# mourisl/T1K

Hardware: AMD Instinct MI355X
Metric: genotyped reads/sec (end-to-end genotyper stage, 2x150 bp HLA) (higher is better)
Workload: dtype u64

## Files before the change

### t1k_amd/csrc/t1k_assign.hip

```cpp
#include "t1k_dev.h"
#include "t1k_launch.h"
#include "t1k_memo.h"

#define WG 256
#define GA_BIG_MAX 2048
#define GA_SCRATCH_INTS (6 * (GA_BIG_MAX + 4))

enum { ERR_HITCAP = 1, ERR_STAGECAP = 2, ERR_CANDCAP = 4, ERR_BIGGROUP = 8, ERR_OVLCAP = 16, ERR_SORTCAP = 32, ERR_SLOWCAP = 64, ERR_ROWCAP = 128, ERR_GROUPCAP = 256 };

__global__ void k_pack_reads(const char *ascii, const uint64_t *offs, uint32_t n, int S, uint64_t *bases, uint64_t *nmask, uint16_t *lens, int nCode) {
  uint64_t gid = (uint64_t)blockIdx.x * blockDim.x + threadIdx.x;
  uint64_t total = (uint64_t)n * S;
  if (gid >= total) return;
  uint32_t re = (uint32_t)(gid / S);
  int w = (int)(gid % S);
  uint64_t o = offs[re];
  int len = (int)(offs[re + 1] - o);
  if (w == 0) lens[re] = (uint16_t)len;
  uint64_t fb = 0, fn = 0, rb = 0, rn = 0;
  for (int q = 0; q < 32; ++q) {
    int i = w * 32 + q;
    if (i >= len) break;
    char c = ascii[o + i];
    int code = c == 'A' ? 0 : c == 'C' ? 1 : c == 'G' ? 2 : c == 'T' ? 3 : 4;
// ... 338 lines not shown
#define SEL_F_EXTOK 2u
#define SEL_F_KEEPCLIP 4u
__device__ __forceinline__ bool packSelectKey(const KeyW &W, int m, int d, int rspan, uint32_t allele, uint32_t index, uint32_t flags, int aBits, int iBits, uint64_t *out) {
  const int MMAX = (1 << W.MB) - 1, DMAX = (1 << W.DB) - 1, RMAX = (1 << W.RB) - 1;
  if (m < 0 || m > MMAX || d < 0 || d > DMAX || rspan < 0 || rspan > RMAX || 1 + W.MB + W.DB + W.RB + 3 + aBits + iBits > 64) return false;
  *out = ((((((uint64_t)(MMAX - m) << W.DB | (uint64_t)d) << W.RB | (uint64_t)(RMAX - rspan)) << aBits | (uint64_t)allele) << iBits) | (uint64_t)index) << 3 | flags;
  return true;
}

__device__ inline bool candBeforeFull(const T1kCand &a, const T1kCand &b) {
  int ars = a.readSE & 0xFFFF, are = a.readSE >> 16, brs = b.readSE & 0xFFFF, bre = b.readSE >> 16;
  if (ars != brs) return ars < brs;
  if (are != bre) return are < bre;
  if (a.seqStart != b.seqStart) return a.seqStart < b.seqStart;
  return a.seqEnd < b.seqEnd;
}

#define SELECT_SMALL 2048
#define SELECT_LARGE 8192

#ifndef T1K_SELECT_SMALL_WAVES
#define T1K_SELECT_SMALL_WAVES 7
#endif
template <int SELECT_LDS_CAP, int NT, bool XL>
__global__ __launch_bounds__(NT) __attribute__((amdgpu_waves_per_eu(SELECT_LDS_CAP == SELECT_SMALL ? T1K_SELECT_SMALL_WAVES : 8))) void k_select(SelectArgs P) {
  extern __shared__ uint64_t dynLds[];
  uint64_t *sKey = dynLds;
  __shared__ uint32_t warpSums[NT / 64];
  __shared__ int sLatch, sGood, sBest, sTie;
  __shared__ uint32_t sBase;
  __shared__ CsTables sCs;
  __shared__ uint16_t sCnt[256 * (NT / 64)];
  const int tid = threadIdx.x;
  unsigned int nbTotal = 0;
  __shared__ uint32_t sNextRe;
  uint32_t hoNext = 0, hoLeft = 0;
  for (;;) {
    __syncthreads();
    if (tid == 0) {
      constexpr uint32_t HO = SELECT_LDS_CAP == SELECT_SMALL ? T1K_SELECT_SMALL_HANDOUT : T1K_SELECT_LARGE_HANDOUT;
      if (hoLeft == 0) { hoNext = (uint32_t)atomicAdd(&P.counters[SELECT_LDS_CAP == SELECT_SMALL ? 28 : 29], (unsigned long long)HO); hoLeft = HO; }
      sNextRe = hoNext++; --hoLeft;
    }
    __syncthreads();
    const uint32_t re = sNextRe;
    if (re >= P.reads.nReadEnds) break;
    const uint32_t n = P.candCount[re], c0 = P.candStart[re];
    if (n == 0) {
      if (tid == 0 && SELECT_LDS_CAP == SELECT_SMALL) { P.ovlStart[re] = 0; P.ovlCount[re] = 0; }
      continue;
    }
    if ((n > SELECT_SMALL) != (SELECT_LDS_CAP == SELECT_LARGE)) continue;
    const uint32_t live = n;
    if (live == 0) {
      if (tid == 0) { P.ovlStart[re] = 0; P.ovlCount[re] = 0; }
      continue;
    }
    uint32_t np2 = 8;
    while (np2 < live) np2 <<= 1;
    uint64_t *key;
    if (np2 <= SELECT_LDS_CAP) key = sKey;
    else if (np2 <= P.sortCap) key = P.sortScratch + (uint64_t)blockIdx.x * P.sortCap * 6;
    else {
      if (tid == 0) { atomicOr(&P.counters[2], (unsigned long long)ERR_SORTCAP); P.ovlStart[re] = 0; P.ovlCount[re] = 0; }
      continue;
    }
    int iBits = 1;
    while ((1u << iBits) < n) ++iBits;
    const uint64_t iMask = (1ull << iBits) - 1;
    const KeyW W = selectWidths<XL>((int)P.reads.len[re]);
    const int mShift = W.DB + W.RB + P.alleleBits + iBits + 3;
    const int mMax = (1 << W.MB) - 1;
    auto idxOf = [&](uint64_t kk) { return (uint32_t)((kk >> 3) & iMask); };
    auto seedOf = [&](uint64_t kk) { return mMax - (int)((kk >> mShift) & (uint64_t)mMax); };
    for (uint32_t i = live + tid; i < np2; i += NT) key[i] = ~0ull;
    for (uint32_t i = tid; i < n; i += NT) {
      const uint16_t fl = P.ext[c0 + i].flags;
      const T1kCand c = P.cand[c0 + i];
      int rs = c.readSE & 0xFFFF, rend = c.readSE >> 16;
      int m = (int)(c.match >> 16);
      int rspan = rend - rs, d = rspan + 1 + c.seqEnd - c.seqStart + 1;
      const double sim = (double)m / (double)(c.seqEnd - c.seqStart + 1 + rend - rs + 1);
      const uint32_t kf = ((fl & T1K_F_SEPSEED) ? SEL_F_SEPSEED : 0u) | ((fl & T1K_F_EXTOK) ? SEL_F_EXTOK : 0u) |
                          (((fl & T1K_F_NEEDCLIP) && !(sim < 0.95)) ? SEL_F_KEEPCLIP : 0u);
      const uint32_t slot = i;
      uint64_t kk;
      if (!packSelectKey(W, m, d, rspan, c.allele & 0x7FFFFFFFu, i, kf, P.alleleBits, iBits, &kk)) { atomicOr(&P.counters[2], (unsigned long long)ERR_SORTCAP); kk = (uint64_t)i << 3; }
// ... 42 lines not shown
    __syncthreads();
    if (tid == 0) sGood = sFirst == 0x7FFFFFFF ? -1 : seedOf(key[sFirst]);
    __syncthreads();
    const int good = sGood;
    uint32_t written = 0;
    unsigned int nbLocal = 0;
    int myBest = -1;
    uint32_t mine = 0;
    for (uint32_t i = tid; i < live; i += NT) {
      const uint64_t kk = key[i];
      const uint32_t fl = (uint32_t)kk & 7u;
      bool emit = false;
      if (!(fl & SEL_F_SEPSEED)) {
        bool tried = true;
        if ((int)i > latch && seedOf(kk) < good && !(fl & SEL_F_KEEPCLIP)) tried = false;
        emit = tried && (fl & SEL_F_EXTOK);
        if (emit) { const int xm = (int)P.ext[c0 + idxOf(kk)].matchCnt; if (xm > myBest) myBest = xm; }
      }
      if (emit) { ++mine; key[i] = kk | (1ull << 63); }
    }
    atomicMax(&sBest, myBest);
    uint32_t tot;
    t1k_block_scan_exclusive_n<NT / 64>(mine, warpSums, &tot);
    if (tid == 0) {
      unsigned long long b = atomicAdd(&P.counters[1], (unsigned long long)tot);
      if (b + tot > P.ovlCap) { atomicOr(&P.counters[2], (unsigned long long)ERR_OVLCAP); sBase = 0xFFFFFFFFu; P.ovlStart[re] = 0; P.ovlCount[re] = 0; }
      else { sBase = (uint32_t)b; P.ovlStart[re] = (uint32_t)b; P.ovlCount[re] = tot; }
    }
    __syncthreads();
    const int bestMatch = sBest;
    if (sBase != 0xFFFFFFFFu) {
      for (uint32_t i0 = 0; i0 < live; i0 += NT) {
        uint32_t i = i0 + tid;
        uint32_t flag = (i < live && (key[i] >> 63)) ? 1u : 0u;
        uint32_t t2;
        uint32_t off = t1k_block_scan_exclusive_n<NT / 64>(flag, warpSums, &t2);
        if (flag) {
          uint32_t ci = c0 + idxOf(key[i]);
          const T1kCand c = P.cand[ci];
          const T1kExt x = P.ext[ci];
          T1kOvl o;
          o.allele = c.allele & 0x7FFFFFFFu;
          o.seqStart = x.seqStart; o.seqEnd = x.seqEnd; o.readStart = x.readStart; o.readEnd = x.readEnd;
          o.matchCnt = x.matchCnt; o.leftClip = x.leftClip; o.rightClip = x.rightClip; o.re = re;
          o.flags = ((int)x.matchCnt >= bestMatch - 10 ? 1u : 0u) | ((c.allele >> 31) ? 0u : 2u);
          o.relaxed = (!P.relax && (o.flags & 1)) ? x.matchCnt : (uint16_t)0;
          if (o.flags & 1) ++nbLocal;
          P.ovl[(uint64_t)sBase + written + off] = o;
        }
        written += t2;
      }
    }
    nbTotal += nbLocal;
    __syncthreads();
  }
  t1k_stat_add(P.counters, T1K_STAT_NEARBEST, nbTotal);
}


__global__ __launch_bounds__(WG) void k_fullalign(FullArgs P) {
  uint64_t gid = (uint64_t)blockIdx.x * blockDim.x + threadIdx.x;
  if (gid >= P.nOvl) return;
  T1kOvl o = P.ovl[gid];
  if (!(o.flags & 1)) { P.ovl[gid].relaxed = 0; return; }
  const int pass = (o.flags & 2) ? 1 : 0;
  const int S = P.reads.S;
  const uint64_t *rb = P.reads.bases + ((uint64_t)o.re * 2 + pass) * S;
  const uint64_t *rn = P.reads.nmask + ((uint64_t)o.re * 2 + pass) * S;
  const int64_t goff = (int64_t)P.ref.alleleOff[o.allele];
  const int L = o.readEnd - o.readStart + 1, Ls = o.seqEnd - o.seqStart + 1;
  const int w = P.noCov ? 0 : (P.undo ? -(int)P.reads.weight[o.re] : (int)P.reads.weight[o.re]);
  bool slow = (L != Ls) || L > T1K_MAX_READ_LEN;
  int x = 0, exonMis = 0;
  uint64_t covw[10];
  if (!slow && L <= 160) {
    typedef uint64_t u64x2 __attribute__((ext_vector_type(2), aligned(8)));
    uint64_t gB[6], gN[6], rB[6], rN[6], gE[6];
    const int64_t gpos = goff + o.seqStart;
// ... 447 lines not shown
    __syncthreads();
    if (threadIdx.x == 0) sCarry += (int32_t)tot;
    __syncthreads();
  }
}

int t1k_launch_pack(t1k_ctx *ctx, const char *dAscii, const uint64_t *dOffs, uint32_t n, int S, uint64_t *bases, uint64_t *nmask, uint16_t *lens, int nCode) {
  uint64_t total = (uint64_t)n * S;
  if (!total) return 0;
  hipLaunchKernelGGL(k_pack_reads, dim3((unsigned)((total + 255) / 256)), dim3(256), 0, ctx->stream, dAscii, dOffs, n, S, bases, nmask, lens, nCode);
  return 0;
}

size_t t1k_slow_per_thread(int maxCells) { return (size_t)GA_SCRATCH_INTS * 4 + 4224 + (size_t)maxCells + 64; }

void t1k_launch_extend(t1k_ctx *ctx, const ExtendArgs &a) {
  if (!a.nCand) return;
  hipLaunchKernelGGL(k_extend, dim3((unsigned)((a.nCand + WG - 1) / WG)), dim3(WG), 0, ctx->stream, a);
}
void t1k_launch_extend_retry_dev(t1k_ctx *ctx, const ExtendArgs &a, const uint32_t *list, int arena, uint64_t est) {
  const unsigned long long *nDev = (const unsigned long long *)ctx->bCounters.p + T1K_TOTAL_BASE + arena;
  hipLaunchKernelGGL(k_extend_retry, dim3((unsigned)std::max<uint64_t>(1, (est + WG - 1) / WG)), dim3(WG), 0, ctx->stream, a, list, 0u, nDev);
}
void t1k_launch_select(t1k_ctx *ctx, const SelectArgs &a, int nWg) {
  if (a.xl) {
    hipFuncSetAttribute((const void *)k_select<SELECT_LARGE, 1024, true>, hipFuncAttributeMaxDynamicSharedMemorySize, SELECT_LARGE * 8);
    hipLaunchKernelGGL((k_select<SELECT_SMALL, 256, true>), dim3(nWg), dim3(256), SELECT_SMALL * 8, ctx->stream, a);
    hipLaunchKernelGGL((k_select<SELECT_LARGE, 1024, true>), dim3(std::min(nWg, 512)), dim3(1024), SELECT_LARGE * 8, ctx->stream, a);
    return;
  }
  hipFuncSetAttribute((const void *)k_select<SELECT_LARGE, 1024, false>, hipFuncAttributeMaxDynamicSharedMemorySize, SELECT_LARGE * 8);
  hipLaunchKernelGGL((k_select<SELECT_SMALL, 256, false>), dim3(nWg), dim3(256), SELECT_SMALL * 8, ctx->stream, a);
  hipLaunchKernelGGL((k_select<SELECT_LARGE, 1024, false>), dim3(std::min(nWg, 512)), dim3(1024), SELECT_LARGE * 8, ctx->stream, a);
}
void t1k_launch_fullalign(t1k_ctx *ctx, const FullArgs &a) {
  if (!a.nOvl) return;
  hipLaunchKernelGGL(k_fullalign, dim3((unsigned)((a.nOvl + WG - 1) / WG)), dim3(WG), 0, ctx->stream, a);
}
void t1k_launch_fullalign_slow(t1k_ctx *ctx, const SlowArgs &a, int nBlocks) { hipLaunchKernelGGL(k_fullalign_slow, dim3(nBlocks * 64), dim3(64), 0, ctx->stream, a); }
void t1k_launch_align_flags(t1k_ctx *ctx, const SlowArgs &a, uint32_t *flags) {
  hipLaunchKernelGGL(k_align_flags, dim3((a.nSlow + WG - 1) / WG), dim3(WG), 0, ctx->stream, a, flags);
}
void t1k_launch_align_reps(t1k_ctx *ctx, const uint32_t *flags, const uint32_t *runOf, uint32_t *rep, uint32_t n) {
  hipLaunchKernelGGL(k_align_reps, dim3((n + WG - 1) / WG), dim3(WG), 0, ctx->stream, flags, runOf, rep, n);
}
void t1k_launch_align_fill_apply(t1k_ctx *ctx, const SlowArgs &a, bool eq) {
  if (eq) {
    hipLaunchKernelGGL(k_align_fill<true>, dim3((a.nRuns + WG - 1) / WG), dim3(WG), 0, ctx->stream, a);
    hipLaunchKernelGGL(k_align_apply_eq, dim3((a.nSlow + WG - 1) / WG), dim3(WG), 0, ctx->stream, a);
  } else {
    hipLaunchKernelGGL(k_align_fill<false>, dim3((a.nRuns + WG - 1) / WG), dim3(WG), 0, ctx->stream, a);
    hipLaunchKernelGGL(k_align_apply_band, dim3((a.nSlow + WG - 1) / WG), dim3(WG), 0, ctx->stream, a);
  }
}
void t1k_launch_truncate(t1k_ctx *ctx, const TruncArgs &a, int nWg) {
  if (a.xl) {
// ... 96 lines not shown
```

### t1k_amd/csrc/t1k_capi.hip

```cpp
#include <sys/mman.h>
#include <map>
#include <mutex>
#include <unordered_map>
#include <algorithm>
#include <memory>
#include <thread>
#include <chrono>
#include <cstring>
#include <cstdio>
#include <cstdlib>
#include "t1k_dev.h"
#include "t1k_launch.h"

namespace {
struct DevPool {
  std::mutex m;
  std::map<int, std::multimap<size_t, void *>> freeBlocks;
  std::unordered_map<void *, std::pair<size_t, int>> live;
  size_t pooled = 0;
};
DevPool &devPool() { static DevPool *p = new DevPool(); return *p; }
}

hipError_t t1k_dev_malloc(void **out, size_t bytes) {
// ... 754 lines not shown
      const uint64_t before = ctx->wGroup;
      grow(ctx->wGroup, ctx->needGroup, ctx->prm.group_cap);
      if (ctx->wGroup > before && !ctx->scaledOnce) {
        const double f = std::min(4.0, (double)ctx->wGroup / (double)before);
        ctx->wList = std::min<uint64_t>((uint64_t)ctx->prm.group_cap, (uint64_t)(ctx->wList * f));
        ctx->wCand = std::min<uint64_t>((uint64_t)ctx->prm.cand_cap, (uint64_t)(ctx->wCand * f));
        ctx->wOvl = std::min<uint64_t>((uint64_t)ctx->prm.ovl_cap, (uint64_t)(ctx->wOvl * f));
        ctx->scaledOnce = true;
      }
      grow(ctx->wList, ctx->needList, ctx->prm.group_cap);
      grow(ctx->wRare, ctx->needRare, ctx->prm.group_cap);
      grow(ctx->wJob, ctx->needJob, jobLimit * 2);
      grow(ctx->wGenJob, ctx->needGenJob, jobLimit * 2);
    }
    if (ctx->lastCapFlags & 2) grow(ctx->wGenHit, ctx->needGenHit, genHitLimit);
    if (ctx->lastCapFlags & 4) grow(ctx->wCand, ctx->needCand, ctx->prm.cand_cap);
    if (ctx->lastCapFlags & 16) grow(ctx->wOvl, ctx->needOvl, ctx->prm.ovl_cap);
    if (ctx->lastCapFlags & 64) grew = true;
    if (!grew || (ctx->lastCapFlags & ~(256ull | 4ull | 16ull | 64ull | 2ull))) return rc;
    if (getenv("T1K_DEBUG_PHASES")) fprintf(stderr, "[t1k] range of %u read-ends again with capacities: groups %llu lists %llu / %llu jobs %llu / %llu candidates %llu overlaps %llu\n", count,
                                            (unsigned long long)ctx->wGroup, (unsigned long long)ctx->wList, (unsigned long long)ctx->wRare, (unsigned long long)ctx->wJob, (unsigned long long)ctx->wGenJob,
                                            (unsigned long long)ctx->wCand, (unsigned long long)ctx->wOvl);
  }
}

static int assignOnce(t1k_ctx *ctx, uint64_t first, uint32_t count) {
  const uint32_t n = count;
  ctx->covCommitted = false;
  T1kReadsDev rd = ctx->reads;
  rd.nReadEnds = count;
  rd.bases += first * 2 * rd.S; rd.nmask += first * 2 * rd.S; rd.len += first; rd.weight += first;
  if (rd.skip) rd.skip += first;
  ctx->rangeCount = count;
  int rc;
  const int nWg = (int)std::min<uint32_t>((uint32_t)ctx->prm.workgroups, std::max<uint32_t>(n, 1));
  const uint32_t sortCap = 1u << 15;
  const int maxChunks = t1k_chain_max_chunks(ctx->ref.nAlleles), memoN = t1k_chain_memo_entries();
  const bool longReads = ctx->batchFastMaxLen > 160;
  const int recStride = t1k_chain_rec_stride(ctx->batchFastMaxLen);
  const uint64_t groupCap = ctx->wGroup;
  const uint32_t jobCap = (uint32_t)ctx->wJob, genCandCap = 16u << 20, genHitCap = (uint32_t)std::min<uint64_t>(ctx->wGenHit ? ctx->wGenHit : (64u << 20), 1024u << 20), genJobCap = (uint32_t)ctx->wGenJob;
  const int bigBlocks = 32;
  if ((rc = t1k_ensure(ctx, ctx->bCounters, (size_t)T1K_COUNTER_WORDS * 8))) return rc;
  if ((rc = t1k_ensure(ctx, ctx->bWgGroups, groupCap * recStride * 4))) return rc;
  if ((rc = t1k_ensure(ctx, ctx->bWgStage, (size_t)n * maxChunks * 8 + 64))) return rc;
  const int maxK = t1k_chain_max_kmers(ctx->batchMaxLen, ctx->prm.kmer_length);
// ... 5 lines not shown
  const uint32_t jobSegCap = jobCap / T1K_NSTRIPE, genCandSegCap = genCandCap / T1K_NSTRIPE;
  const size_t listWords = (size_t)listSegCap * T1K_NSTRIPE, rareWords = (size_t)rareSegCap * T1K_NSTRIPE;
  if ((rc = t1k_ensure(ctx, ctx->bLists, ((size_t)jobCap * 2 + listWords * 5 + rareWords * 6 + (size_t)genCandCap * 6 + genHitCap + (size_t)genJobCap * 2) * 4 + 64))) return rc;
  if ((rc = t1k_ensure(ctx, ctx->bCand, (size_t)ctx->wCand * sizeof(T1kCand)))) return rc;
  if ((rc = t1k_ensure(ctx, ctx->bExt, (size_t)ctx->wCand * sizeof(T1kExt)))) return rc;
  const uint64_t chunkEntries = std::max<uint64_t>(ctx->wOvl, (uint64_t)std::max(1, ctx->prm.store_chunk_mb) * ((1ull << 20) / sizeof(T1kOvlP)));
  {
    const int sl = ctx->storeSlot;
    std::vector<T1kDevBuf> &chunks = ctx->storeChunks[sl];
    for (;;) {
      if (ctx->storeChunk[sl] >= chunks.size()) chunks.resize(ctx->storeChunk[sl] + 1);
      T1kDevBuf &ch = chunks[ctx->storeChunk[sl]];
      if (ch.p && ctx->storeUsed[sl] + ctx->wOvl <= ch.bytes / sizeof(T1kOvlP)) break;
      if (ch.p && ctx->storeUsed[sl] > 0) { ++ctx->storeChunk[sl]; ctx->storeUsed[sl] = 0; continue; }
      if (ch.p) { (void)t1k_dev_free(ch.p); ch.p = nullptr; ch.bytes = 0; }
      const auto t0 = std::chrono::steady_clock::now();
      hipError_t e = t1k_dev_malloc(&ch.p, chunkEntries * sizeof(T1kOvlP));
      ctx->msAlloc += std::chrono::duration<double, std::milli>(std::chrono::steady_clock::now() - t0).count(); ctx->bytesAlloc += chunkEntries * sizeof(T1kOvlP);
      if (e != hipSuccess) { ch.p = nullptr; return t1k_fail(ctx, T1K_ERR_DEVICE, std::string("overlap store: hipMalloc of another ") + std::to_string(chunkEntries * sizeof(T1kOvlP) >> 20) + " MB chunk failed (" + hipGetErrorString(e) + "); fewer fragments per window (T1K_WINDOW) need less"); }
      ch.bytes = chunkEntries * sizeof(T1kOvlP);
    }
    ctx->storeBase = (T1kOvlP *)chunks[ctx->storeChunk[sl]].p + ctx->storeUsed[sl];
  }
  if ((rc = t1k_ensure(ctx, ctx->bOvlWork, (size_t)ctx->wOvl * sizeof(T1kOvl)))) return rc;
  ctx->ovlBase = (T1kOvl *)ctx->bOvlWork.p;
  if ((rc = t1k_ensure(ctx, ctx->bCandStart, (size_t)(n + 1) * 4))) return rc;
  if ((rc = t1k_ensure(ctx, ctx->bCandCount, (size_t)(n + 1) * 4))) return rc;
  if ((rc = t1k_ensure(ctx, ctx->bOvlStart, (size_t)(n + 1) * 4))) return rc;
  if ((rc = t1k_ensure(ctx, ctx->bOvlCount, (size_t)(n + 1) * 4))) return rc;
  if ((rc = t1k_ensure(ctx, ctx->bSortScratch, (size_t)std::min(nWg, 512) * sortCap * 48))) return rc;
  T1K_HIP(ctx, hipMemsetAsync(ctx->bCounters.p, 0, (size_t)T1K_COUNTER_WORDS * 8, ctx->stream));
  T1K_HIP(ctx, hipMemsetAsync(ctx->bOvlCount.p, 0, (size_t)n * 4 + 4, ctx->stream));
  T1K_HIP(ctx, hipMemsetAsync(ctx->bCandCount.p, 0, (size_t)n * 4 + 4, ctx->stream));
  T1K_HIP(ctx, hipMemsetAsync(ctx->bWgCache.p, 0, (size_t)n * memoN * 8, ctx->stream));
  ctx->nCand = ctx->nOvl = 0;
  ctx->traceFetch = 0;
  if (getenv("T1K_DEBUG_TRACE")) fprintf(stderr, "[t1k trace] assign_range first %llu count %u\n", (unsigned long long)first, n);
  memset(&ctx->stats, 0, sizeof(ctx->stats));
  if (n == 0) return T1K_OK;
  unsigned long long hc[64];
  double t0 = nowMs();
  ChainArgs a{};
  a.ref = ctx->ref; a.reads = rd;
  a.k = ctx->prm.kmer_length; a.radius = ctx->prm.radius; a.hitLenRequired = ctx->prm.hit_len_required;
  a.sim = ctx->prm.ref_seq_similarity;
  const int relaxFlag = ctx->prm.relax_intron_align;
  a.recs = (uint32_t *)ctx->bWgGroups.p; a.recStride = (uint32_t)recStride; a.groupCap = groupCap;
  a.chunkStart = (uint32_t *)ctx->bWgStage.p; a.chunkCount = a.chunkStart + (size_t)n * maxChunks; a.maxChunks = maxChunks;
// ... 22 lines not shown
  ctx->nCand = hc[0];
  ExtendArgs e{};
  e.ref = ctx->ref; e.reads = rd; e.k = a.k; e.sim = a.sim;
  e.cand = a.cand; e.ext = (T1kExt *)ctx->bExt.p; e.nCand = ctx->nCand; e.counters = a.counters;
  e.memo = a.memo; e.jobStr = a.jobStr; e.jobSegCap = a.jobSegCap; e.retryStr = a.retryStr; e.retrySegCap = a.listSegCap;
  t1k_launch_extend(ctx, e);
  if (ctx->nCand) {
    const uint64_t jobCapAll = (uint64_t)e.jobSegCap * T1K_NSTRIPE, retryCapAll = (uint64_t)e.retrySegCap * T1K_NSTRIPE;
    const uint64_t eJ = t1k_arena_estimate(ctx, T1K_AR_EXTJOBS, jobCapAll, n), eR = t1k_arena_estimate(ctx, T1K_AR_EXTRETRY, retryCapAll, n);
    t1k_arena_compact_dev(ctx, T1K_AR_EXTJOBS, e.jobStr, e.jobSegCap, a.jobList, eJ);
    t1k_arena_compact_dev(ctx, T1K_AR_EXTRETRY, e.retryStr, e.retrySegCap, a.retryList, eR);
    t1k_launch_dp_dense_dev(ctx, a, a.jobList, T1K_AR_EXTJOBS, (uint32_t)jobCapAll, eJ);
    t1k_launch_extend_retry_dev(ctx, e, a.retryList, T1K_AR_EXTRETRY, eR);
  }
  T1K_HIP(ctx, hipEventRecord(ctx->ev[2], ctx->stream));
  double t2 = nowMs();
  SelectArgs s{};
  s.reads = rd; s.cand = a.cand; s.ext = e.ext; s.candStart = a.candStart; s.candCount = a.candCount;
  s.ovl = ctx->ovlBase; s.ovlCap = ctx->wOvl;
  s.ovlStart = (uint32_t *)ctx->bOvlStart.p; s.ovlCount = (uint32_t *)ctx->bOvlCount.p;
  s.sortScratch = (uint64_t *)ctx->bSortScratch.p; s.sortCap = sortCap; s.counters = a.counters;
  s.alleleBits = 1; s.relax = relaxFlag; s.xl = ctx->batchMaxLen > T1K_MAX_READ_LEN ? 1 : 0;
  while ((1u << s.alleleBits) < ctx->ref.nAlleles) ++s.alleleBits;
  t1k_launch_select(ctx, s, nWg);
  T1K_HIP(ctx, hipEventRecord(ctx->ev[3], ctx->stream));
  if ((rc = fetchCounters(ctx, hc))) return rc;
  double t3 = nowMs();
  if (hc[2]) return capacityError(ctx, hc[2]);
  t1k_arena_estimate_set(ctx, T1K_AR_EXTJOBS, t1k_arena_counts(ctx, T1K_AR_EXTJOBS, e.jobSegCap).total, n);
  t1k_arena_estimate_set(ctx, T1K_AR_EXTRETRY, t1k_arena_counts(ctx, T1K_AR_EXTRETRY, e.retrySegCap).total, n);
  ctx->nOvl = hc[1];
  const bool deferCov = ctx->covMode == 1;
  if (relaxFlag || !deferCov) {
    if (!deferCov) ctx->covCommitted = true;
    if ((rc = t1k_fullalign_phase(ctx, rd, s.ovl, ctx->nOvl, relaxFlag, deferCov ? 1 : 0, ctx->batchMaxLen, false, hc))) return rc;
  } else {
    T1K_HIP(ctx, hipEventRecord(ctx->ev[7], ctx->stream));
    hc[8] = hc[15] = hc[20] = 0;
  }
  hipEvent_t evSlow = ctx->ev[9];
  T1K_HIP(ctx, hipEventRecord(evSlow, ctx->stream));
  TruncArgs tr{};
  tr.reads = rd; tr.ovl = s.ovl; tr.ovlStart = s.ovlStart; tr.ovlCount = s.ovlCount; tr.sortScratch = s.sortScratch; tr.sortCap = sortCap; tr.alleleBits = s.alleleBits;
  tr.counters = a.counters; tr.xl = s.xl;
  t1k_launch_truncate(ctx, tr, nWg);
  T1K_HIP(ctx, hipEventRecord(ctx->ev[4], ctx->stream));
  t1k_launch_publish_lists(ctx, rd.listPtr + first, rd.listCount + first, ctx->ovlBase, ctx->storeBase, ctx->nOvl, s.ovlStart, s.ovlCount, n, a.counters, rd.skip);
  if ((rc = fetchCounters(ctx, hc))) return rc;
  double t4 = nowMs();
  if (hc[2]) return capacityError(ctx, hc[2]);
  ctx->storeUsed[ctx->storeSlot] += ctx->nOvl;
  if (getenv("T1K_DEBUG_PHASES")) {
    float a1 = 0, a2 = 0, a3 = 0;
    (void)hipEventElapsedTime(&a1, ctx->ev[3], ctx->ev[7]); (void)hipEventElapsedTime(&a2, ctx->ev[7], evSlow); (void)hipEventElapsedTime(&a3, evSlow, ctx->ev[4]);
    fprintf(stderr, "[t1k] fullalign %.2f ms, eq-DP (%llu jobs) + general-DP (%llu jobs) %.2f ms, truncate %.2f ms; cand %llu ovl %llu dp %llu; groups %llu (gap walk %llu) fast %llu general %llu big %llu; memo jobs %llu parked %llu wide-queue %llu\n",
            a1, hc[8], hc[15], a2, a3, hc[0], hc[1], hc[7], hc[6], (unsigned long long)ctx->lastSlowGroups, hc[11], hc[12], hc[13], hc[16], hc[17], hc[20]);
#ifdef T1K_NEAR_STATS
    fprintf(stderr, "[t1k] multi-diagonal groups: far strays %llu, near count saturated %llu, other fallback %llu, masks ok but not a chain (<= 32 hits) %llu, (> 32 hits) %llu, chain (<= 96) %llu, chain (> 96) %llu\n", hc[40], hc[41], hc[42], hc[43], hc[47], hc[45], hc[46]);
#endif
#ifdef T1K_WALK_STATS
    fprintf(stderr, "[t1k] gap walk classes: exact without a DP %llu, pruned by the per-gap bound %llu, memo / DP %llu\n", hc[40], hc[41], hc[42]);
#endif
  }
  t1k_stats &st = ctx->stats;
  st.read_ends = n; st.lookups = hc[3]; st.postings = hc[4]; st.hits = hc[5]; st.groups = hc[6]; st.candidates = hc[0]; st.extended = hc[1];
  st.dp_calls = hc[7] + hc[14]; st.near_best = hc[10]; st.dp_cells = hc[24];
  float ms[4] = {0, 0, 0, 0}, msSeed = 0;
  for (int i = 0; i < 4; ++i) (void)hipEventElapsedTime(&ms[i], ctx->ev[i], ctx->ev[i + 1]);
  (void)hipEventElapsedTime(&msSeed, ctx->ev[0], ctx->ev[8]);
  (void)t1; (void)t2; (void)t3;
  st.ms_seed = msSeed; st.ms_chain = ms[0] - msSeed; st.ms_extend = ms[1]; st.ms_select = ms[2]; st.ms_fullalign = ms[3]; st.ms_total = t4 - t0;
  st.batches = 1;
  return T1K_OK;
}

int t1k_overlaps_download(t1k_ctx *ctx, uint32_t *counts, t1k_overlap *out, uint64_t cap, uint64_t *total) {
  if (!ctx) return T1K_ERR_ARG;
  T1K_HIP(ctx, hipSetDevice(ctx->device));
  const uint32_t n = ctx->rangeCount;
  std::vector<uint32_t> start(n), cnt(n);
  if (n) {
    T1K_HIP(ctx, hipMemcpy(start.data(), ctx->bOvlStart.p, (size_t)n * 4, hipMemcpyDeviceToHost));
    T1K_HIP(ctx, hipMemcpy(cnt.data(), ctx->bOvlCount.p, (size_t)n * 4, hipMemcpyDeviceToHost));
  }
  uint64_t tot = 0;
  for (uint32_t i = 0; i < n; ++i) tot += cnt[i];
  if (total) *total = tot;
  if (counts) memcpy(counts, cnt.data(), (size_t)n * 4);
  if (!out) return T1K_OK;
  if (cap < tot) return t1k_fail(ctx, T1K_ERR_ARG, "overlap buffer too small");
  std::vector<T1kOvl> h(ctx->nOvl);
  if (ctx->nOvl) T1K_HIP(ctx, hipMemcpy(h.data(), ctx->ovlBase, ctx->nOvl * sizeof(T1kOvl), hipMemcpyDeviceToHost));
  uint64_t w = 0;
  for (uint32_t i = 0; i < n; ++i) {
    for (uint32_t j = 0; j < cnt[i]; ++j) {
      const T1kOvl &o = h[(uint64_t)start[i] + j];
      t1k_overlap &r = out[w++];
      r.seq_idx = (int32_t)o.allele; r.read_start = o.readStart; r.read_end = o.readEnd; r.seq_start = o.seqStart; r.seq_end = o.seqEnd;
      r.strand = (o.flags & 2) ? -1 : 1;
      r.match_cnt = o.matchCnt; r.left_clip = o.leftClip; r.right_clip = o.rightClip; r.relaxed_match_cnt = o.relaxed;
      r.similarity = (double)o.matchCnt / (double)(o.readEnd - o.readStart + 1 + o.seqEnd - o.seqStart + 1 + 2 * o.leftClip + 2 * o.rightClip);
    }
  }
  return T1K_OK;
}

int t1k_overlaps_upload(t1k_ctx *ctx, const uint32_t *counts, const t1k_overlap *ovl) {
  if (!ctx || !counts) return t1k_fail(ctx, T1K_ERR_ARG, "t1k_overlaps_upload: bad arguments");
  if (!ctx->ref.bases) return t1k_fail(ctx, T1K_ERR_STATE, "t1k_overlaps_upload: no reference");
  if (!ctx->reads.listPtr || ctx->readsShared) return t1k_fail(ctx, T1K_ERR_STATE, "t1k_overlaps_upload: no read set of this context's own");
  T1K_HIP(ctx, hipSetDevice(ctx->device));
  const uint32_t n = ctx->reads.nReadEnds;
  uint64_t tot = 0;
  for (uint32_t i = 0; i < n; ++i) tot += counts[i];
  if (tot && !ovl) return t1k_fail(ctx, T1K_ERR_ARG, "t1k_overlaps_upload: bad arguments");
// ... 41 lines not shown
```

### t1k_amd/csrc/t1k_dev.h

```cpp
#pragma once
#include <hip/hip_runtime.h>
#include <stdint.h>
#include <string>
#include <type_traits>
#include <vector>
#include "../../include/t1k_gpu.h"

#define T1K_MAX_READ_LEN 320
#define T1K_LONG_READ_LEN 1000
#define T1K_EVEN 0x5555555555555555ull
#define T1K_NEG_BIG (-(1 << 28))

struct T1kPosting { uint32_t allele, offset; };

struct T1kCand {
  uint32_t allele;
  uint32_t readSE;
  int32_t seqStart, seqEnd;
  uint32_t match;
  uint32_t re;
};

struct T1kExt {
  int32_t seqStart, seqEnd;
// ... 738 lines not shown
  hipEvent_t ev[12] = {};
  t1k_params prm;
  std::string err;
  T1kRefDev ref{};
  std::vector<uint64_t> hAlleleOff;
  std::vector<uint32_t> hAlleleLen;
  std::vector<T1kDevBuf> refBufs;
  T1kReadsDev reads{};
  T1kDevBuf bReadAscii, bReadOffs, bReadBases, bReadN, bReadLen, bReadWeight, bListPtr, bListCount;
  T1kDevBuf bDedupScratch, bDedupBases, bDedupN, bDedupLen, bDedupWeight;
  bool readsShared = false;
  int batchMaxLen = 0;
  int batchFastMaxLen = 0;
  int covFullLen = 0;
  bool covFullDirty = false;
  uint32_t rangeCount = 0;
  T1kDevBuf bWgHits, bWgGroups, bWgStage, bWgBig, bWgCache, bLists;
  std::vector<T1kDevBuf> storeChunks[2];
  int storeSlot = 0;
  size_t storeChunk[2] = {0, 0};
  uint64_t storeUsed[2] = {0, 0};
  T1kOvl *ovlBase = nullptr;
  T1kDevBuf bOvlWork;
  T1kDevBuf bOvlUpload;
  T1kOvlP *storeBase = nullptr;
  uint64_t wGroup = 0, wList = 0, wRare = 0, wCand = 0, wOvl = 0, wJob = 0, wGenJob = 0, wGenHit = 0;
  uint64_t needGroup = 0, needList = 0, needRare = 0, needCand = 0, needOvl = 0, needJob = 0, needGenJob = 0, needGenHit = 0;
  unsigned long long lastCapFlags = 0;
  bool scaledOnce = false;
  bool covCommitted = false;
  uint32_t queueBoost = 1;
  int covMode = 0;
  double msAlloc = 0;
  uint64_t bytesAlloc = 0;
  T1kDevBuf bCand, bExt, bCandStart, bCandCount, bOvlStart, bOvlCount, bCounters, bSlowQueue, bSlowScratch, bSortScratch, bEqTrace, bSortTmp, bJobSort;
  uint64_t nCand = 0, nOvl = 0;
  T1kDevBuf bEnd1, bEnd2, bHasN, bRows, bRowStart, bRowCount, bFragAssigned, bPairScratch, bPairOverflow, bPairBig, bExtractHuge;
  uint32_t nFragments = 0;
  uint64_t nRows = 0;
  T1kDevBuf bEmRowPtr, bEmEc, bEmCount, bEmLen, bEmX0, bEmN, bEmPsum, bEmColPtr, bEmRowOf;
  std::vector<uint64_t> emPieceBytes, emPieceDispl;
  uint32_t emGroups = 0, emEc = 0, emRowBegin = 0, emRowEnd = 0;
  struct t1k_comm *emComm = nullptr;
  bool emReduceMode = false;
  uint64_t emNnz = 0;
  std::vector<int32_t> hEmLen;
// ... 43 lines not shown
```

### t1k_amd/csrc/t1k_launch.h

```cpp
#pragma once
#include <algorithm>
#include <mutex>
#include "t1k_dev.h"

#define T1K_USED_MASK_WORDS 10
struct ChainArgs {
  T1kRefDev ref;
  T1kReadsDev reads;
  int k, radius, hitLenRequired;
  double sim;
  uint32_t *recs; uint32_t recStride; uint64_t groupCap;
  uint32_t *chunkStart, *chunkCount; int maxChunks;
  uint32_t *usedMask;
  uint32_t *usedOut, *usedCount;
  unsigned long long *memo;
  uint32_t *jobList; uint32_t jobCap;
  uint32_t *retryList, *generalList, *bigList;
  uint32_t *jobStr, *retryStr, *generalStr, *bigStr, *finishStr, *waveStr, *waveList, *slowStr, *slowList;
  uint32_t groupSegCap, jobSegCap, listSegCap, rareSegCap, genCandSegCap, genHitSegCap;
  uint32_t maxK;
  uint32_t maxKFast;
  uint32_t *genJobStr, *genJobList; uint32_t genJobSegCap;
  uint32_t *genHits;
  uint32_t *genCand; uint32_t genCandCap;
// ... 7 lines not shown
};

struct ExtendArgs {
  T1kRefDev ref;
  T1kReadsDev reads;
  int k;
  double sim;
  const T1kCand *cand;
  T1kExt *ext;
  uint64_t nCand;
  unsigned long long *counters;
  unsigned long long *memo;
  uint32_t *jobStr; uint32_t jobSegCap;
  uint32_t *retryStr; uint32_t retrySegCap;
};

struct SelectArgs {
  T1kReadsDev reads;
  const T1kCand *cand;
  const T1kExt *ext;
  const uint32_t *candStart, *candCount;
  T1kOvl *ovl; uint64_t ovlCap;
  uint32_t *ovlStart, *ovlCount;
  uint64_t *sortScratch;
  uint32_t sortCap;
  int alleleBits;
  int relax;
  int xl;
  unsigned long long *counters;
};

struct FullArgs {
  T1kRefDev ref;
  T1kReadsDev reads;
  int relax;
  int noCov;
  int fullLen;
  int undo;
  T1kOvl *ovl;
  uint64_t nOvl;
  uint32_t *eqStr, *bandStr, *wideStr; uint32_t segCap;
  unsigned long long *eqKeyStr, *bandKeyStr;
  unsigned long long *counters;
};

struct SlowArgs {
// ... 73 lines not shown
inline int t1k_bits(unsigned long long v) {
  int b = 1;
  while (b < 64 && (v >> b)) ++b;
  return b;
}

int t1k_rowset_chunk(t1k_rowset *rs, t1k_ctx *ctx, size_t *chunk, t1k_row_entry **rows, uint64_t *cap, unsigned long long **cursor);
int t1k_rowset_chunk_full(t1k_rowset *rs, t1k_ctx *ctx, size_t chunk);
int t1k_exclusive_sum64(t1k_ctx *ctx, const uint32_t *in, unsigned long long *out, uint32_t n);
int t1k_exclusive_sum32(t1k_ctx *ctx, const uint32_t *in, uint32_t *out, uint64_t n);
int t1k_exclusive_sum_u64(t1k_ctx *ctx, const unsigned long long *in, unsigned long long *out, uint64_t n);

int t1k_launch_pack(t1k_ctx *ctx, const char *dAscii, const uint64_t *dOffs, uint32_t n, int S, uint64_t *bases, uint64_t *nmask, uint16_t *lens, int nCode);
size_t t1k_slow_per_thread(int maxCells);
size_t t1k_chain_big_scratch_u32();
int t1k_chain_max_chunks(uint32_t nAlleles);
int t1k_chain_memo_entries();
int t1k_chain_rec_stride(int maxLen);
int t1k_chain_max_kmers(int maxLen, int k);
int t1k_chain_used_u32(int maxK);
int t1k_launch_seed(t1k_ctx *ctx, const ChainArgs &a, bool longReads, bool xlong);
int t1k_run_chain(t1k_ctx *ctx, const ChainArgs &a, int nWg, int bigBlocks, bool longReads, unsigned long long *hc);
void t1k_launch_extend(t1k_ctx *ctx, const ExtendArgs &a);
void t1k_launch_select(t1k_ctx *ctx, const SelectArgs &a, int nWg);
void t1k_launch_fullalign(t1k_ctx *ctx, const FullArgs &a);
void t1k_launch_fullalign_slow(t1k_ctx *ctx, const SlowArgs &a, int nBlocks);
void t1k_launch_align_flags(t1k_ctx *ctx, const SlowArgs &a, uint32_t *flags);
void t1k_launch_align_reps(t1k_ctx *ctx, const uint32_t *flags, const uint32_t *runOf, uint32_t *rep, uint32_t n);
void t1k_launch_align_fill_apply(t1k_ctx *ctx, const SlowArgs &a, bool eq);
int t1k_inclusive_sum(t1k_ctx *ctx, const uint32_t *in, uint32_t *out, uint64_t n);
void t1k_launch_truncate(t1k_ctx *ctx, const TruncArgs &a, int nWg);
void t1k_launch_coverage_scan(t1k_ctx *ctx, const T1kRefDev &ref, int32_t *out, const uint64_t *outOff);
int t1k_fetch_counters(t1k_ctx *ctx, unsigned long long *h);
int t1k_fullalign_phase(t1k_ctx *ctx, const T1kReadsDev &rd, T1kOvl *ovl, uint64_t nOvl, int relaxFlag, int noCov, int maxLen, bool exactQueues, unsigned long long *hc);
struct T1kArenaCounts { uint64_t total; uint32_t maxSeg; bool overflow; };
T1kArenaCounts t1k_arena_counts(const t1k_ctx *ctx, int arena, uint32_t segCap);
void t1k_launch_coverage_add(t1k_ctx *ctx, int32_t *dst, int32_t *src, uint64_t n);
int t1k_coverage_fold(t1k_ctx *ctx);
void t1k_launch_missing_coverage(t1k_ctx *ctx, const T1kRefDev &ref, int32_t *scratch, int32_t *missing);
void t1k_arena_compact_dev(t1k_ctx *ctx, int arena, const uint32_t *src, uint32_t segCap, uint32_t *dst, uint64_t estTotal);
void t1k_launch_dp_dense_dev(t1k_ctx *ctx, const ChainArgs &a, const uint32_t *jobs, int arena, uint32_t cap, uint64_t est);
uint64_t t1k_arena_estimate(const t1k_ctx *ctx, int arena, uint64_t cap, uint32_t nRe);
void t1k_arena_estimate_set(t1k_ctx *ctx, int arena, uint64_t total, uint32_t nRe);
void t1k_launch_extend_retry_dev(t1k_ctx *ctx, const ExtendArgs &a, const uint32_t *list, int arena, uint64_t est);
void t1k_arena_compact64(t1k_ctx *ctx, int arena, const unsigned long long *src, uint32_t segCap, unsigned long long *dst, uint32_t maxSeg);
int t1k_run_table(t1k_ctx *ctx, const unsigned long long *keys, uint32_t n, const unsigned long long *lone,
                  uint32_t *flag, uint32_t *scan, uint32_t *runStart, unsigned long long *runKey, uint32_t *runs);
// ... 11 lines not shown
```

Baseline: 3.774 million.

## Fuse selection with packed store and truncation, skipping full-align phase when eligible

When intron relaxation is off and coverage mode is 1, the select kernel now writes packed overlap records straight into the store and sets per-read list pointers. This skips the unpacked overlap buffer and the later full-align/truncate/pack phases, and the host returns right after selection. For reads with more than 1000 emitted overlaps, the kernel re-sorts them by a truncation key inside the kernel and cuts the list at the similarity threshold. This removes later kernels, host syncs and a large intermediate buffer, but it assumes full alignment is not needed in this mode and adds a serial tie-break insertion sort on one thread.

```diff
diff --git a/t1k_amd/csrc/t1k_assign.hip b/t1k_amd/csrc/t1k_assign.hip
--- a/t1k_amd/csrc/t1k_assign.hip
+++ b/t1k_amd/csrc/t1k_assign.hip
@@ -384,7 +384,7 @@
 #ifndef T1K_SELECT_SMALL_WAVES
 #define T1K_SELECT_SMALL_WAVES 7
 #endif
-template <int SELECT_LDS_CAP, int NT, bool XL>
+template <int SELECT_LDS_CAP, int NT, bool XL, bool PK>
 __global__ __launch_bounds__(NT) __attribute__((amdgpu_waves_per_eu(SELECT_LDS_CAP == SELECT_SMALL ? T1K_SELECT_SMALL_WAVES : 8))) void k_select(SelectArgs P) {
   extern __shared__ uint64_t dynLds[];
   uint64_t *sKey = dynLds;
@@ -395,6 +395,11 @@
   __shared__ uint16_t sCnt[256 * (NT / 64)];
   const int tid = threadIdx.x;
   unsigned int nbTotal = 0;
+  unsigned long long emitTotal = 0;
+  auto publish = [&](uint32_t re, uint32_t start, uint32_t count) {
+    P.ovlStart[re] = start; P.ovlCount[re] = count;
+    if (PK && !(P.reads.skip && P.reads.skip[re])) { P.listPtr[re] = (unsigned long long)(P.store + start); P.listCount[re] = count; }
+  };
   __shared__ uint32_t sNextRe;
   uint32_t hoNext = 0, hoLeft = 0;
   for (;;) {
@@ -409,13 +414,13 @@
     if (re >= P.reads.nReadEnds) break;
     const uint32_t n = P.candCount[re], c0 = P.candStart[re];
     if (n == 0) {
-      if (tid == 0 && SELECT_LDS_CAP == SELECT_SMALL) { P.ovlStart[re] = 0; P.ovlCount[re] = 0; }
+      if (tid == 0 && SELECT_LDS_CAP == SELECT_SMALL) publish(re, 0, 0);
       continue;
     }
     if ((n > SELECT_SMALL) != (SELECT_LDS_CAP == SELECT_LARGE)) continue;
     const uint32_t live = n;
     if (live == 0) {
-      if (tid == 0) { P.ovlStart[re] = 0; P.ovlCount[re] = 0; }
+      if (tid == 0) publish(re, 0, 0);
       continue;
     }
     uint32_t np2 = 8;
@@ -424,7 +429,7 @@
     if (np2 <= SELECT_LDS_CAP) key = sKey;
     else if (np2 <= P.sortCap) key = P.sortScratch + (uint64_t)blockIdx.x * P.sortCap * 6;
     else {
-      if (tid == 0) { atomicOr(&P.counters[2], (unsigned long long)ERR_SORTCAP); P.ovlStart[re] = 0; P.ovlCount[re] = 0; }
+      if (tid == 0) { atomicOr(&P.counters[2], (unsigned long long)ERR_SORTCAP); publish(re, 0, 0); }
       continue;
     }
     int iBits = 1;
@@ -513,38 +518,133 @@
     atomicMax(&sBest, myBest);
     uint32_t tot;
     t1k_block_scan_exclusive_n<NT / 64>(mine, warpSums, &tot);
+    auto makeOvl = [&](uint32_t ci, int bestMatch) {
+      const T1kCand c = P.cand[ci];
+      const T1kExt x = P.ext[ci];
+      T1kOvl o;
+      o.allele = c.allele & 0x7FFFFFFFu;
+      o.seqStart = x.seqStart; o.seqEnd = x.seqEnd; o.readStart = x.readStart; o.readEnd = x.readEnd;
+      o.matchCnt = x.matchCnt; o.leftClip = x.leftClip; o.rightClip = x.rightClip; o.re = re;
+      o.flags = ((int)x.matchCnt >= bestMatch - 10 ? 1u : 0u) | ((c.allele >> 31) ? 0u : 2u);
+      o.relaxed = (!P.relax && (o.flags & 1)) ? x.matchCnt : (uint16_t)0;
+      return o;
+    };
+    auto storePacked = [&](uint64_t at, const T1kOvl &o) {
+      T1kOvlP p;
+      if (!t1k_ovl_pack(o, p)) atomicOr(&P.counters[2], 1024ull);
+      P.store[at] = p;
+    };
+    uint32_t keep = tot;
+    const bool cutList = PK && tot > 1000;
+    if (cutList) {
+      __syncthreads();
+      const int bestMatch = sBest;
+      uint32_t *emitBits = (uint32_t *)sCnt;
+      for (uint32_t q = tid; q < (n + 31) / 32; q += NT) emitBits[q] = 0;
+      __syncthreads();
+      for (uint32_t i = tid; i < live; i += NT)
+        if (key[i] >> 63) { const uint32_t ix = idxOf(key[i]); atomicOr(&emitBits[ix >> 5], 1u << (ix & 31)); }
+      __syncthreads();
+      const KeyW TW = truncWidths<XL>((int)P.reads.len[re]);
+      uint32_t done = 0;
+      for (uint32_t i0 = 0; i0 < n; i0 += NT) {
+        const uint32_t i = i0 + tid;
+        const bool flag = i < n && ((emitBits[i >> 5] >> (i & 31)) & 1u);
+        uint64_t kk = 0;
+        if (flag) {
+          const T1kExt x = P.ext[c0 + i];
+          const int rspan = x.readEnd - x.readStart;
+          const int d = rspan + 1 + x.seqEnd - x.seqStart + 1 + 2 * x.leftClip + 2 * x.rightClip;
+          if (!packSortKey(TW, (int)x.matchCnt, d, rspan, P.cand[c0 + i].allele & 0x7FFFFFFFu, i, P.alleleBits, iBits, &kk)) { atomicOr(&P.counters[2], (unsigned long long)ERR_SORTCAP); kk = i; }
+          if ((int)x.matchCnt >= bestMatch - 10) ++nbLocal;
+        }
+        uint32_t t2;
+        const uint32_t off = t1k_block_scan_exclusive_n<NT / 64>(flag ? 1u : 0u, warpSums, &t2);
+        if (flag) key[done + off] = kk;
+        done += t2;
+      }
+      uint32_t np2t = 8;
+      while (np2t < tot) np2t <<= 1;
+      for (uint32_t i = tot + tid; i < np2t; i += NT) key[i] = ~0ull;
+      __syncthreads();
+      if (key != sKey || !ldsClassRanks<NT>(key, tot, P.alleleBits + iBits, sCs)) bitonicSort(key, np2t);
+      else ldsCountingPass<NT>(key, tot, sCnt, warpSums, [&](uint64_t kk) { return csRankOf(sCs, (uint32_t)(kk >> (P.alleleBits + iBits))); });
+      if (tid == 0) { sTie = 0; sLatch = (int)tot; }
+      __syncthreads();
+      for (uint32_t i = 1 + tid; i < tot; i += NT)
+        if ((key[i] >> iBits) == (key[i - 1] >> iBits)) sTie = 1;
+      __syncthreads();
+      if (sTie && tid == 0) {
+        auto before = [&](uint32_t ia, uint32_t ib) {
+          const T1kExt xa = P.ext[c0 + ia], xb = P.ext[c0 + ib];
+          if (xa.readStart != xb.readStart) return xa.readStart < xb.readStart;
+          if (xa.readEnd != xb.readEnd) return xa.readEnd < xb.readEnd;
+          if (xa.seqStart != xb.seqStart) return xa.seqStart < xb.seqStart;
+          if (xa.seqEnd != xb.seqEnd) return xa.seqEnd < xb.seqEnd;
+          const T1kCand a = P.cand[c0 + ia], b = P.cand[c0 + ib];
+          const int ma = (int)(a.match >> 16), mb = (int)(b.match >> 16);
+          if (ma != mb) return ma > mb;
+          const int ra = (int)(a.readSE >> 16) - (int)(a.readSE & 0xFFFF), rb = (int)(b.readSE >> 16) - (int)(b.readSE & 0xFFFF);
+          const int da = ra + 1 + a.seqEnd - a.seqStart + 1, db = rb + 1 + b.seqEnd - b.seqStart + 1;
+          if (da != db) return da < db;
+          if (ra != rb) return ra > rb;
+          if (candBeforeFull(a, b)) return true;
+          if (candBeforeFull(b, a)) return false;
+          return ia < ib;
+        };
+        for (uint32_t i = 1; i < tot; ++i) {
+          if ((key[i] >> iBits) != (key[i - 1] >> iBits)) continue;
+          uint32_t j = i;
+          while (j > 0 && (key[j - 1] >> iBits) == (key[j] >> iBits) && before((uint32_t)(key[j] & iMask), (uint32_t)(key[j - 1] & iMask))) {
+            uint64_t t = key[j]; key[j] = key[j - 1]; key[j - 1] = t;
+            --j;
+          }
+        }
+      }
+      __syncthreads();
+      {
+        const int tmMax = (1 << TW.MB) - 1, tdMax = (1 << TW.DB) - 1, dShift = TW.RB + P.alleleBits + iBits;
+        auto simOf = [&](uint64_t kk) { return (double)(tmMax - (int)((kk >> (dShift + TW.DB)) & (uint64_t)tmMax)) / (double)(int)((kk >> dShift) & (uint64_t)tdMax); };
+        const double s0 = simOf(key[0]);
+        uint32_t first = tot;
+        for (uint32_t j = 1 + tid; j < tot; j += NT)
+          if (simOf(key[j]) < s0 - 0.1) { first = j; break; }
+        if (first < tot) atomicMin(&sLatch, (int)first);
+      }
+      __syncthreads();
+      keep = (uint32_t)sLatch;
+    }
     if (tid == 0) {
-      unsigned long long b = atomicAdd(&P.counters[1], (unsigned long long)tot);
-      if (b + tot > P.ovlCap) { atomicOr(&P.counters[2], (unsigned long long)ERR_OVLCAP); sBase = 0xFFFFFFFFu; P.ovlStart[re] = 0; P.ovlCount[re] = 0; }
-      else { sBase = (uint32_t)b; P.ovlStart[re] = (uint32_t)b; P.ovlCount[re] = tot; }
+      unsigned long long b = atomicAdd(&P.counters[1], (unsigned long long)keep);
+      emitTotal += tot;
+      if (b + keep > P.ovlCap) { atomicOr(&P.counters[2], (unsigned long long)ERR_OVLCAP); sBase = 0xFFFFFFFFu; publish(re, 0, 0); }
+      else { sBase = (uint32_t)b; publish(re, (uint32_t)b, keep); }
     }
     __syncthreads();
     const int bestMatch = sBest;
     if (sBase != 0xFFFFFFFFu) {
-      for (uint32_t i0 = 0; i0 < live; i0 += NT) {
-        uint32_t i = i0 + tid;
-        uint32_t flag = (i < live && (key[i] >> 63)) ? 1u : 0u;
-        uint32_t t2;
-        uint32_t off = t1k_block_scan_exclusive_n<NT / 64>(flag, warpSums, &t2);
-        if (flag) {
-          uint32_t ci = c0 + idxOf(key[i]);
-          const T1kCand c = P.cand[ci];
-          const T1kExt x = P.ext[ci];
-          T1kOvl o;
-          o.allele = c.allele & 0x7FFFFFFFu;
-          o.seqStart = x.seqStart; o.seqEnd = x.seqEnd; o.readStart = x.readStart; o.readEnd = x.readEnd;
-          o.matchCnt = x.matchCnt; o.leftClip = x.leftClip; o.rightClip = x.rightClip; o.re = re;
-          o.flags = ((int)x.matchCnt >= bestMatch - 10 ? 1u : 0u) | ((c.allele >> 31) ? 0u : 2u);
-          o.relaxed = (!P.relax && (o.flags & 1)) ? x.matchCnt : (uint16_t)0;
-          if (o.flags & 1) ++nbLocal;
-          P.ovl[(uint64_t)sBase + written + off] = o;
+      if (cutList) {
+        for (uint32_t i = tid; i < keep; i += NT) storePacked((uint64_t)sBase + i, makeOvl(c0 + (uint32_t)(key[i] & iMask), bestMatch));
+      } else {
+        for (uint32_t i0 = 0; i0 < live; i0 += NT) {
+          uint32_t i = i0 + tid;
+          uint32_t flag = (i < live && (key[i] >> 63)) ? 1u : 0u;
+          uint32_t t2;
+          uint32_t off = t1k_block_scan_exclusive_n<NT / 64>(flag, warpSums, &t2);
+          if (flag) {
+            const T1kOvl o = makeOvl(c0 + idxOf(key[i]), bestMatch);
+            if (o.flags & 1) ++nbLocal;
+            if (PK) storePacked((uint64_t)sBase + written + off, o);
+            else P.ovl[(uint64_t)sBase + written + off] = o;
+          }
+          written += t2;
         }
-        written += t2;
       }
     }
     nbTotal += nbLocal;
     __syncthreads();
   }
+  if (PK && tid == 0 && emitTotal) atomicAdd(&P.counters[21], emitTotal);
   t1k_stat_add(P.counters, T1K_STAT_NEARBEST, nbTotal);
 }
 
@@ -1038,16 +1138,15 @@
   const unsigned long long *nDev = (const unsigned long long *)ctx->bCounters.p + T1K_TOTAL_BASE + arena;
   hipLaunchKernelGGL(k_extend_retry, dim3((unsigned)std::max<uint64_t>(1, (est + WG - 1) / WG)), dim3(WG), 0, ctx->stream, a, list, 0u, nDev);
 }
-void t1k_launch_select(t1k_ctx *ctx, const SelectArgs &a, int nWg) {
-  if (a.xl) {
-    hipFuncSetAttribute((const void *)k_select<SELECT_LARGE, 1024, true>, hipFuncAttributeMaxDynamicSharedMemorySize, SELECT_LARGE * 8);
-    hipLaunchKernelGGL((k_select<SELECT_SMALL, 256, true>), dim3(nWg), dim3(256), SELECT_SMALL * 8, ctx->stream, a);
-    hipLaunchKernelGGL((k_select<SELECT_LARGE, 1024, true>), dim3(std::min(nWg, 512)), dim3(1024), SELECT_LARGE * 8, ctx->stream, a);
-    return;
-  }
-  hipFuncSetAttribute((const void *)k_select<SELECT_LARGE, 1024, false>, hipFuncAttributeMaxDynamicSharedMemorySize, SELECT_LARGE * 8);
-  hipLaunchKernelGGL((k_select<SELECT_SMALL, 256, false>), dim3(nWg), dim3(256), SELECT_SMALL * 8, ctx->stream, a);
-  hipLaunchKernelGGL((k_select<SELECT_LARGE, 1024, false>), dim3(std::min(nWg, 512)), dim3(1024), SELECT_LARGE * 8, ctx->stream, a);
+template <bool XL, bool PK>
+static void launchSelect(t1k_ctx *ctx, const SelectArgs &a, int nWg) {
+  hipFuncSetAttribute((const void *)k_select<SELECT_LARGE, 1024, XL, PK>, hipFuncAttributeMaxDynamicSharedMemorySize, SELECT_LARGE * 8);
+  hipLaunchKernelGGL((k_select<SELECT_SMALL, 256, XL, PK>), dim3(nWg), dim3(256), SELECT_SMALL * 8, ctx->stream, a);
+  hipLaunchKernelGGL((k_select<SELECT_LARGE, 1024, XL, PK>), dim3(std::min(nWg, 512)), dim3(1024), SELECT_LARGE * 8, ctx->stream, a);
+}
+void t1k_launch_select(t1k_ctx *ctx, const SelectArgs &a, int nWg, bool packed) {
+  if (a.xl) { if (packed) launchSelect<true, true>(ctx, a, nWg); else launchSelect<true, false>(ctx, a, nWg); }
+  else { if (packed) launchSelect<false, true>(ctx, a, nWg); else launchSelect<false, false>(ctx, a, nWg); }
 }
 void t1k_launch_fullalign(t1k_ctx *ctx, const FullArgs &a) {
   if (!a.nOvl) return;
diff --git a/t1k_amd/csrc/t1k_capi.hip b/t1k_amd/csrc/t1k_capi.hip
--- a/t1k_amd/csrc/t1k_capi.hip
+++ b/t1k_amd/csrc/t1k_capi.hip
@@ -800,6 +800,18 @@
                                             (unsigned long long)ctx->wGroup, (unsigned long long)ctx->wList, (unsigned long long)ctx->wRare, (unsigned long long)ctx->wJob, (unsigned long long)ctx->wGenJob,
                                             (unsigned long long)ctx->wCand, (unsigned long long)ctx->wOvl);
   }
+}
+
+static int finishRangeStats(t1k_ctx *ctx, uint32_t n, const unsigned long long *hc, unsigned long long emitted, double t0) {
+  t1k_stats &st = ctx->stats;
+  st.read_ends = n; st.lookups = hc[3]; st.postings = hc[4]; st.hits = hc[5]; st.groups = hc[6]; st.candidates = hc[0]; st.extended = emitted;
+  st.dp_calls = hc[7] + hc[14]; st.near_best = hc[10]; st.dp_cells = hc[24];
+  float ms[4] = {0, 0, 0, 0}, msSeed = 0;
+  for (int i = 0; i < 4; ++i) (void)hipEventElapsedTime(&ms[i], ctx->ev[i], ctx->ev[i + 1]);
+  (void)hipEventElapsedTime(&msSeed, ctx->ev[0], ctx->ev[8]);
+  st.ms_seed = msSeed; st.ms_chain = ms[0] - msSeed; st.ms_extend = ms[1]; st.ms_select = ms[2]; st.ms_fullalign = ms[3]; st.ms_total = nowMs() - t0;
+  st.batches = 1;
+  return T1K_OK;
 }
 
 static int assignOnce(t1k_ctx *ctx, uint64_t first, uint32_t count) {
@@ -851,8 +863,10 @@
     }
     ctx->storeBase = (T1kOvlP *)chunks[ctx->storeChunk[sl]].p + ctx->storeUsed[sl];
   }
-  if ((rc = t1k_ensure(ctx, ctx->bOvlWork, (size_t)ctx->wOvl * sizeof(T1kOvl)))) return rc;
-  ctx->ovlBase = (T1kOvl *)ctx->bOvlWork.p;
+  const bool packedSelect = !ctx->prm.relax_intron_align && ctx->covMode == 1;
+  if (!packedSelect && (rc = t1k_ensure(ctx, ctx->bOvlWork, (size_t)ctx->wOvl * sizeof(T1kOvl)))) return rc;
+  ctx->ovlBase = packedSelect ? nullptr : (T1kOvl *)ctx->bOvlWork.p;
+  ctx->ovlPacked = packedSelect;
   if ((rc = t1k_ensure(ctx, ctx->bCandStart, (size_t)(n + 1) * 4))) return rc;
   if ((rc = t1k_ensure(ctx, ctx->bCandCount, (size_t)(n + 1) * 4))) return rc;
   if ((rc = t1k_ensure(ctx, ctx->bOvlStart, (size_t)(n + 1) * 4))) return rc;
@@ -921,8 +935,20 @@
   s.sortScratch = (uint64_t *)ctx->bSortScratch.p; s.sortCap = sortCap; s.counters = a.counters;
   s.alleleBits = 1; s.relax = relaxFlag; s.xl = ctx->batchMaxLen > T1K_MAX_READ_LEN ? 1 : 0;
   while ((1u << s.alleleBits) < ctx->ref.nAlleles) ++s.alleleBits;
-  t1k_launch_select(ctx, s, nWg);
+  s.store = ctx->storeBase; s.listPtr = rd.listPtr + first; s.listCount = rd.listCount + first;
+  t1k_launch_select(ctx, s, nWg, packedSelect);
   T1K_HIP(ctx, hipEventRecord(ctx->ev[3], ctx->stream));
+  if (packedSelect) {
+    T1K_HIP(ctx, hipEventRecord(ctx->ev[4], ctx->stream));
+    if ((rc = fetchCounters(ctx, hc))) return rc;
+    if (hc[2]) return capacityError(ctx, hc[2]);
+    t1k_arena_estimate_set(ctx, T1K_AR_EXTJOBS, t1k_arena_counts(ctx, T1K_AR_EXTJOBS, e.jobSegCap).total, n);
+    t1k_arena_estimate_set(ctx, T1K_AR_EXTRETRY, t1k_arena_counts(ctx, T1K_AR_EXTRETRY, e.retrySegCap).total, n);
+    ctx->nOvl = hc[1];
+    ctx->storeUsed[ctx->storeSlot] += ctx->nOvl;
+    if (getenv("T1K_DEBUG_PHASES")) fprintf(stderr, "[t1k] packed selection: cand %llu emitted %llu kept %llu\n", hc[0], hc[21], hc[1]);
+    return finishRangeStats(ctx, n, hc, hc[21], t0);
+  }
   if ((rc = fetchCounters(ctx, hc))) return rc;
   double t3 = nowMs();
   if (hc[2]) return capacityError(ctx, hc[2]);
@@ -961,16 +987,8 @@
     fprintf(stderr, "[t1k] gap walk classes: exact without a DP %llu, pruned by the per-gap bound %llu, memo / DP %llu\n", hc[40], hc[41], hc[42]);
 #endif
   }
-  t1k_stats &st = ctx->stats;
-  st.read_ends = n; st.lookups = hc[3]; st.postings = hc[4]; st.hits = hc[5]; st.groups = hc[6]; st.candidates = hc[0]; st.extended = hc[1];
-  st.dp_calls = hc[7] + hc[14]; st.near_best = hc[10]; st.dp_cells = hc[24];
-  float ms[4] = {0, 0, 0, 0}, msSeed = 0;
-  for (int i = 0; i < 4; ++i) (void)hipEventElapsedTime(&ms[i], ctx->ev[i], ctx->ev[i + 1]);
-  (void)hipEventElapsedTime(&msSeed, ctx->ev[0], ctx->ev[8]);
-  (void)t1; (void)t2; (void)t3;
-  st.ms_seed = msSeed; st.ms_chain = ms[0] - msSeed; st.ms_extend = ms[1]; st.ms_select = ms[2]; st.ms_fullalign = ms[3]; st.ms_total = t4 - t0;
-  st.batches = 1;
-  return T1K_OK;
+  (void)t1; (void)t2; (void)t3; (void)t4;
+  return finishRangeStats(ctx, n, hc, hc[1], t0);
 }
 
 int t1k_overlaps_download(t1k_ctx *ctx, uint32_t *counts, t1k_overlap *out, uint64_t cap, uint64_t *total) {
@@ -989,7 +1007,11 @@
   if (!out) return T1K_OK;
   if (cap < tot) return t1k_fail(ctx, T1K_ERR_ARG, "overlap buffer too small");
   std::vector<T1kOvl> h(ctx->nOvl);
-  if (ctx->nOvl) T1K_HIP(ctx, hipMemcpy(h.data(), ctx->ovlBase, ctx->nOvl * sizeof(T1kOvl), hipMemcpyDeviceToHost));
+  if (ctx->ovlPacked) {
+    std::vector<T1kOvlP> hp(ctx->nOvl);
+    if (ctx->nOvl) T1K_HIP(ctx, hipMemcpy(hp.data(), ctx->storeBase, ctx->nOvl * sizeof(T1kOvlP), hipMemcpyDeviceToHost));
+    for (uint64_t g = 0; g < ctx->nOvl; ++g) h[g] = t1k_ovl_unpack(hp[g]);
+  } else if (ctx->nOvl) T1K_HIP(ctx, hipMemcpy(h.data(), ctx->ovlBase, ctx->nOvl * sizeof(T1kOvl), hipMemcpyDeviceToHost));
   uint64_t w = 0;
   for (uint32_t i = 0; i < n; ++i) {
     for (uint32_t j = 0; j < cnt[i]; ++j) {
diff --git a/t1k_amd/csrc/t1k_dev.h b/t1k_amd/csrc/t1k_dev.h
--- a/t1k_amd/csrc/t1k_dev.h
+++ b/t1k_amd/csrc/t1k_dev.h
@@ -784,6 +784,7 @@
   uint64_t storeUsed[2] = {0, 0};
   T1kOvl *ovlBase = nullptr;
   T1kDevBuf bOvlWork;
+  bool ovlPacked = false;
   T1kDevBuf bOvlUpload;
   T1kOvlP *storeBase = nullptr;
   uint64_t wGroup = 0, wList = 0, wRare = 0, wCand = 0, wOvl = 0, wJob = 0, wGenJob = 0, wGenHit = 0;
diff --git a/t1k_amd/csrc/t1k_launch.h b/t1k_amd/csrc/t1k_launch.h
--- a/t1k_amd/csrc/t1k_launch.h
+++ b/t1k_amd/csrc/t1k_launch.h
@@ -53,6 +53,9 @@
   const uint32_t *candStart, *candCount;
   T1kOvl *ovl; uint64_t ovlCap;
   uint32_t *ovlStart, *ovlCount;
+  T1kOvlP *store;
+  unsigned long long *listPtr;
+  uint32_t *listCount;
   uint64_t *sortScratch;
   uint32_t sortCap;
   int alleleBits;
@@ -172,7 +175,7 @@
 int t1k_launch_seed(t1k_ctx *ctx, const ChainArgs &a, bool longReads, bool xlong);
 int t1k_run_chain(t1k_ctx *ctx, const ChainArgs &a, int nWg, int bigBlocks, bool longReads, unsigned long long *hc);
 void t1k_launch_extend(t1k_ctx *ctx, const ExtendArgs &a);
-void t1k_launch_select(t1k_ctx *ctx, const SelectArgs &a, int nWg);
+void t1k_launch_select(t1k_ctx *ctx, const SelectArgs &a, int nWg, bool packed);
 void t1k_launch_fullalign(t1k_ctx *ctx, const FullArgs &a);
 void t1k_launch_fullalign_slow(t1k_ctx *ctx, const SlowArgs &a, int nBlocks);
 void t1k_launch_align_flags(t1k_ctx *ctx, const SlowArgs &a, uint32_t *flags);
```

Measured after the change: 3.867 million, median of 6. +2.5%, better.
